# madsjulia/GeostatInversion.jl

Measured on AMD Instinct MI355X. Metric: randSVD GB/s + top-k singular-value rel-err, n=1e6 rank=256, higher is better.
Workload: dtype f64

## Files before the change

geostatinversion.jl_amd/csrc/hip_backend.hip:

```cpp
#include <hip/hip_runtime.h>
#include <rccl/rccl.h>
#include <dlfcn.h>
#include <fcntl.h>
#include <sched.h>
#include <sys/mman.h>
#include <time.h>
#include <unistd.h>
#include <algorithm>
#include <cmath>
#include <cstdlib>
#include <cstring>
#include <condition_variable>
#include <atomic>
#include <mutex>
#include <string>
#include <chrono>
#include <map>
#include <memory>
#include <set>
#include <vector>
#include "../../include/gsi_hip.h"
#include "backend.hpp"
#include "hip_common.hpp"
#include "host_staging.hpp"
// ... 368 lines not shown
      int64_t cur[3] = {1, 1, 1};
      for (int a = 0; a < d; ++a) cur[a] = 2 * p->N[a];
      int64_t tot = cur[0] * cur[1] * cur[2];
      struct Hold { HipBackend* be; double* p; ~Hold() { if (p) be->release(p); } } bufh{this, nullptr};
      bufh.p = alloc((size_t)tot);
      double*& buf = bufh.p;
      hipk::fft_spectrum_natural(st_, buf, cur, beta, 1);
      auto rotate_apply = [&](int64_t rows_out, int64_t period, bool weighted) {
        const int64_t k = cur[0], rest = (tot / k);
        Hold Bh{this, alloc((size_t)k * rows_out)};
        double* B = Bh.p;
        if (!weighted) hipk::fft_cos_matrix(st_, B, k, rows_out, period, false);
        else hipk::fft_cos_matrix(st_, B, k, rows_out, period, true);
        Hold outh{this, alloc((size_t)rest * rows_out)};
        double* out = outh.p;
        double* ws = gemm_ws(hipk::gemm_workspace_doubles(rest, rows_out, k));
        hipk::gemm_f64(st_, true, rest, rows_out, k, 1.0, buf, k, B, k, 0.0, out, rest, ws);
        check_launch("fft re-embedding product");
        release(buf);
        buf = out;
        outh.p = nullptr;
        tot = rest * rows_out;
        int64_t nd[3] = {1, 1, 1};
        for (int a = 0; a + 1 < d; ++a) nd[a] = cur[a + 1];
        nd[d - 1] = rows_out;
        for (int a = 0; a < 3; ++a) cur[a] = nd[a];
      };
      for (int a = 0; a < d; ++a) rotate_apply(p->N[a], 2 * p->N[a], false);
      for (int a = 0; a < d; ++a) rotate_apply(p->M[a], p->M[a], true);
      hipk::fft_lines_layout(st_, buf, p->lam, p->M);
      hipk::fft_finish_plan(st_, p->lam, p->lam + Mtot, p->M);
      check_launch("fft re-embedded spectrum");
      release(buf);
      buf = nullptr;
    } catch (...) {
      release(p->W); release(p->lam);
      throw;
    }
    return p.release();
  }
  void fftcov_destroy(void* plan) override {
    FftCov* p = static_cast<FftCov*>(plan);
    if (!p) return;
    release(p->W); release(p->lam);
    delete p;
  }
  void fftcov_apply(void* plan, int64_t l, const double* X, int64_t ldx, double* Y, int64_t ldy) override {
    bind();
    FftCov* p = static_cast<FftCov*>(plan);
    hipk::fft_cov_apply(st_, p->N, p->M, p->lam, reinterpret_cast<double2*>(p->W), p->nb_max, l, X, ldx, Y, ldy);
    check_launch("fft_cov_apply");
  }

  void lu_L(double* Y, int64_t m, int64_t l, int64_t ld, int32_t* ipiv_host) override {
    lu_L_impl(Y, m, l, ld, ipiv_host, nullptr);
  }
  bool lu_L_keep(double* Y, int64_t m, int64_t l, int64_t ld, int32_t** ipiv_dev) override {
    if (ipiv_dev == nullptr) return false;
    lu_L_impl(Y, m, l, ld, nullptr, ipiv_dev);
    return true;
  }
  void lu_L_impl(double* Y, int64_t m, int64_t l, int64_t ld, int32_t* ipiv_host, int32_t** ipiv_dev_out) {
    bind();
    hipk::Lu2Work w2;
    static const bool tall_first = (getenv("GSI_LU_TALL") != nullptr && getenv("GSI_LU_TALL")[0] == '1');
    static const int64_t ov_max = getenv("GSI_LU_OV_MAX") ? atoll(getenv("GSI_LU_OV_MAX")) : ((int64_t)5 << 20);
    static const bool ov_off = (getenv("GSI_LU_OV") != nullptr && getenv("GSI_LU_OV")[0] == '0');
    const bool resident_ok = !tall_first && !lu2_lost_ && ranks_sharing_device_ <= 1;
    bool fits = resident_ok && hipk::lu2_config(m, ncus_, &w2.bs, &w2.rpt, &w2.grid) && lu2_fits(w2.bs, w2.rpt, w2.grid);
    if (!fits && resident_ok && !ov_off && m <= ov_max && ncus_ >= 1) {
      const int g = std::min(ncus_, 256);
      if (m > (int64_t)g * 4096) {
        if (lu2_ov_resident_ < 0) lu2_ov_resident_ = hipk::lu2_resident_per_cu_ov();
        if ((int64_t)lu2_ov_resident_ * ncus_ >= g) { w2.bs = 512; w2.rpt = 8; w2.grid = g; w2.ov = true; fits = true; }
      }
    }
    if (fits) {
      if (const char* e = getenv("GSI_LU_POLL_LIMIT")) w2.poll_limit = atoi(e);
      if (const char* e = getenv("GSI_LU_TEST_MUTE_EPOCH")) w2.mute_epoch = (uint32_t)atoi(e);
      if (const char* e = getenv("GSI_LU_COOPERATIVE")) w2.cooperative = (e[0] == '1');
      static const int nb_env = getenv("GSI_LU_NB") ? atoi(getenv("GSI_LU_NB")) : 0;
      w2.nb = (nb_env == 32 || nb_env == 64) ? nb_env : hipk::LU2_NB;
      const size_t rec_bytes = sizeof(unsigned long long) * 2 * ((size_t)w2.grid + hipk::LU2_RES_COPIES) * hipk::LU2_REC_GRANULES;
      const size_t u12_bytes = sizeof(double) * (size_t)w2.nb * (size_t)l;
      grow(ws_lu_, rec_bytes + u12_bytes + sizeof(int32_t) * (l + 4) + 256);
      char* base = (char*)ws_lu_.p;
      w2.recs = (unsigned long long*)base; base += rec_bytes;
      w2.u12 = (double*)base; base += u12_bytes;
      w2.ipiv = (int32_t*)base;
      w2.info = flags_ + 0;
      hipk::lu2_L(st_, Y, m, l, ld, w2);
      check_launch("lu2_L");
      if (ipiv_dev_out) *ipiv_dev_out = w2.ipiv;
      if (ipiv_host) {
        HIP_CHECK(hipMemcpyAsync(ipiv_host, w2.ipiv, sizeof(int32_t) * l, hipMemcpyDeviceToHost, st_));
        HIP_CHECK(hipStreamSynchronize(st_));
      }
      return;
    }
    if (m >= ((int64_t)1 << 31)) throw Error(GSI_ERR_ARG, "lu: panels of 2^31 rows and more are not supported");
    grow(ws_lu_, hipk::lu3_work_bytes(l));
    int32_t* ipiv_dev = nullptr;
    hipk::lu3_L(st_, Y, m, l, ld, ws_lu_.p, flags_ + 0, &ipiv_dev);
    check_launch("lu3_L");
    if (ipiv_dev_out) *ipiv_dev_out = ipiv_dev;
    if (ipiv_host) {
      HIP_CHECK(hipMemcpyAsync(ipiv_host, ipiv_dev, sizeof(int32_t) * l, hipMemcpyDeviceToHost, st_));
      HIP_CHECK(hipStreamSynchronize(st_));
    }
  }
  int lus_block() const override { return hipk::LU2_NB; }
  struct LusWs { double* pval; int64_t* pidx; int32_t* ipiv; };
  LusWs lus_ws(int64_t, int64_t l) {
    if (l > 8188) throw Error(GSI_ERR_ARG, "sharded lu: sketch width too large");
    grow(ws_lus_, 32768 + 2 * 8 * 1024 + 64);
    char* base = (char*)ws_lus_.p;
    LusWs w;
    w.ipiv = (int32_t*)base;
    w.pval = (double*)(base + 32768);
    w.pidx = (int64_t*)(base + 32768 + 8 * 1024);
    return w;
  }
  void lus_u12_leaf(const double* Yloc, int64_t ld, int64_t row0, int64_t jb, int64_t j0, int w, double* U12) override {
    bind();
    hipk::lus_u12_leaf(st_, Yloc, ld, row0, jb, j0, w, U12);
    check_launch("lus_u12_leaf");
  }
  void lus_pending(double* Yloc, int64_t mloc, int64_t ld, int64_t row0, int64_t jb, int64_t j0, int w,
                   const double* U12) override {
    bind();
    if (mloc > 0) hipk::lus_pending(st_, Yloc, ld, mloc, row0, jb, j0, w, U12);
    check_launch("lus_pending");
  }
  void lus_candidate(const double* Yloc, int64_t mloc, int64_t ld, int64_t row0, int64_t l, int64_t j, double* rec) override {
    bind();
    LusWs w = lus_ws(mloc, l);
    const bool ready = (lus_part_col_ == j && lus_part_Y_ == Yloc && lus_part_mloc_ == mloc);
    lus_part_col_ = -1;
    hipk::lus_candidate(st_, Yloc, ld, mloc, row0, l, j, rec, w.pval, w.pidx, ready);
    check_launch("lus_candidate");
  }
  void lus_apply(double* Yloc, int64_t mloc, int64_t ld, int64_t row0, int64_t m, int64_t l, int64_t j0, int s, int w,
                 const double* recs, int nranks) override {
    bind();
    LusWs ws = lus_ws(mloc, l);
    static const bool fuse = (getenv("GSI_LUS_NO_FUSE") == nullptr);
    const bool next = fuse && (s + 1 < w) && mloc > 0;
    hipk::lus_apply(st_, Yloc, ld, mloc, row0, m, l, j0, s, w, recs, nranks, ws.ipiv, flags_ + 0, next ? ws.pval : nullptr,
                    next ? ws.pidx : nullptr);
    check_launch("lus_apply");
    lus_part_col_ = next ? j0 + s + 1 : -1;
    lus_part_Y_ = Yloc;
    lus_part_mloc_ = mloc;
  }
  void lus_u12_block(const double* Yloc, int64_t ld, int64_t row0, int64_t jb, int b, int64_t c0, int64_t c1,
                     double* U12) override {
    bind();
    hipk::lus_u12_block(st_, Yloc, ld, row0, jb, b, c0, c1, U12);
    check_launch("lus_u12_block");
  }
  void lus_rankk(double* Yloc, int64_t mloc, int64_t ld, int64_t row0, int64_t jb, int b, int64_t c0, int64_t t,
                 const double* U12) override {
    bind();
    hipk::lus_rankk(st_, Yloc, ld, mloc, row0, jb, b, c0, t, U12);
    check_launch("lus_rankk");
  }
  void lus_finish(double* Yloc, int64_t mloc, int64_t ld, int64_t row0, int64_t l) override {
// ... 1262 lines not shown
```

geostatinversion.jl_amd/csrc/panel_lu_leaf.hip:

```cpp
#include "hip_common.hpp"
#include <type_traits>
#include <cstdio>
#include <cstdlib>

namespace gsi { namespace hipk {

namespace {

constexpr int LW = LU2_LEAF;
constexpr int KPMAX = LU2_NB - LW;
constexpr int LSP = KPMAX + 1;
constexpr int REC = LU2_REC_GRANULES;
constexpr int POLL_LIMIT = 4000000;

__device__ inline double readlane_d(double x, int srclane) {
  int lo = __double2loint(x), hi = __double2hiint(x);
  lo = __builtin_amdgcn_readlane(lo, srclane);
  hi = __builtin_amdgcn_readlane(hi, srclane);
  return __hiloint2double(hi, lo);
}
template <int CTRL, int ROW_MASK>
__device__ inline double dpp_fmax(double v) {
  const int lo = __builtin_amdgcn_update_dpp(0, __double2loint(v), CTRL, ROW_MASK, 0xf, false);
  const int hi = __builtin_amdgcn_update_dpp((int)0xbff00000, __double2hiint(v), CTRL, ROW_MASK, 0xf, false);
// ... 651 lines not shown
    if (hit) {
#pragma unroll
      for (int rr = 0; rr < R; ++rr)
        if (grow0 + rr * BS == r) {
#pragma unroll
          for (int k = 0; k < LW; ++k) a[rr][k] = c_old[k];
        }
    }
#pragma unroll
    for (int rr = 0; rr < R; ++rr) {
      const double x0 = a[rr][s];
      const double lij = (rpiv != 0.0) ? x0 * rpiv : x0;
      a[rr][s] = lij;
#pragma unroll
      for (int k = s + 1; k < LW; ++k) a[rr][k] -= lij * u[k];
    }
    if (isdiag && tid >= s) {
      if (tid == s) {
#pragma unroll
        for (int k = 0; k < LW; ++k) d[k] = u[k];
      } else {
        if (drow == r) {
#pragma unroll
          for (int k = 0; k < LW; ++k) d[k] = c_old[k];
        }
        const double x0 = d[s];
        const double lij = (rpiv != 0.0) ? x0 * rpiv : x0;
        d[s] = lij;
#pragma unroll
        for (int k = s + 1; k < LW; ++k) d[k] -= lij * u[k];
      }
    }
    LU_STAMP(5);
  };

  {
    using std::integral_constant;
    step(integral_constant<int, 0>{});
    step(integral_constant<int, 1>{});
    step(integral_constant<int, 2>{});
    step(integral_constant<int, 3>{});
    step(integral_constant<int, 4>{});
    step(integral_constant<int, 5>{});
    step(integral_constant<int, 6>{});
    step(integral_constant<int, 7>{});
  }
  if constexpr (OV) {
    for (int32_t i = ov0; i < m; i += ovstride) {
      const int lev = ov_level(i);
      double x[LW];
#pragma unroll
      for (int k = 0; k < LW; ++k) x[k] = (k < w) ? *elem(colbase(j0 + k), i) : 0.0;
#pragma unroll
      for (int t = 0; t < LW; ++t) {
        if (t >= lev && t < w) {
          const double rp = s_rp[t];
          const double lt = (rp != 0.0) ? x[t] * rp : x[t];
          x[t] = lt;
#pragma unroll
          for (int k = t + 1; k < LW; ++k) x[k] -= lt * s_u[t * LW + k];
        }
      }
#pragma unroll
      for (int k = 0; k < LW; ++k) if (k < w) *elem(colbase(j0 + k), i) = x[k];
    }
  }
  if (s_abort && tid == 0) atomicExch(info, -1);
  if (has_col && pend) { swcol[pj] = pa1; swcol[pr] = pa0; }
#pragma unroll
  for (int k = 0; k < LW; ++k) {
    if (k < w) {
      char* cb = colbase(j0 + k);
#pragma unroll
      for (int rr = 0; rr < R; ++rr) {
        const int32_t i = row0 + rr * BS;
        if (i < m) *elem(cb, i) = a[rr][k];
      }
      if (isdiag && drow < m) *elem(cb, drow) = d[k];
    }
  }
}

template <int K>
__global__ __launch_bounds__(256) void lu_u12_kernel(const double* __restrict__ Y, int64_t ld, int64_t jb, int64_t jbrow,
                                                     int64_t c0, int64_t c1, double* __restrict__ out) {
  __shared__ double L11[K * K];
#pragma unroll 8
  for (int e = threadIdx.x; e < K * K; e += 256) {
    const int r = e % K, c = e / K;
    L11[r * K + c] = Y[(jbrow + r) + (jb + c) * ld];
  }
  __syncthreads();
  if (threadIdx.x >= 64) return;
  const int64_t c = c0 + (int64_t)blockIdx.x * 64 + threadIdx.x;
  if (c >= c1) return;
  double x[K];
  const double* col = Y + jbrow + c * ld;
#pragma unroll
  for (int r = 0; r < K; ++r) x[r] = col[r];
#pragma unroll
  for (int r = 1; r < K; ++r) {
    double v = x[r];
#pragma unroll
    for (int p = 0; p < r; ++p) v -= L11[r * K + p] * x[p];
    x[r] = v;
  }
  double* o = out + (c - c0) * K;
#pragma unroll
  for (int r = 0; r < K; ++r) o[r] = x[r];
}

template <int K, int DEPTH, int RK_CHUNK>
__global__ __launch_bounds__(256) __attribute__((amdgpu_waves_per_eu(RK_CHUNK == 64 ? 3 : 2, RK_CHUNK == 64 ? 3 : 4))) void lu_rankk_kernel(double* __restrict__ Y, int64_t ld, int64_t m, int64_t r_begin,
                                                       int64_t jb, int64_t c0, int64_t t,
                                                       const double* __restrict__ U12) {
  typedef double double4_t __attribute__((ext_vector_type(4)));
  constexpr int KP = K + 2;
  extern __shared__ double us[];
  const int tid = threadIdx.x, lane = tid & 63, wave = tid >> 6;
  const int jl = lane & 15, kk = lane >> 4;
  const int64_t rb = r_begin + ((int64_t)blockIdx.x * 4 + wave) * 32;
  double fa[2][K / 4];
#pragma unroll
  for (int h = 0; h < 2; ++h) {
    const int64_t rrow = rb + 16 * h + jl;
#pragma unroll
    for (int s = 0; s < K / 4; ++s) fa[h][s] = (rrow < m) ? Y[rrow + (jb + 4 * s + kk) * ld] : 0.0;
  }
  for (int64_t cc0 = 0; cc0 < t; cc0 += RK_CHUNK) {
    const int tc = (int)((t - cc0 < RK_CHUNK) ? (t - cc0) : RK_CHUNK);
    __syncthreads();
    for (int e = tid; e < RK_CHUNK * K; e += 256) {
      const int k = e % K, c = e / K;
      us[c * KP + k] = (c < tc) ? U12[k + (cc0 + c) * K] : 0.0;
    }
    __syncthreads();
    if (rb >= m) continue;
    const int ntile = (tc + 15) / 16;
    double cin[2][4];
    auto load_tile = [&](int tt, double (&dst)[2][4]) {
#pragma unroll
      for (int h = 0; h < 2; ++h) {
        const int64_t rrow = rb + 16 * h + jl;
#pragma unroll
        for (int reg = 0; reg < 4; ++reg) {
          const int cl = 16 * tt + kk + 4 * reg;
          dst[h][reg] = (rrow < m && cl < tc) ? Y[rrow + (c0 + cc0 + cl) * ld] : 0.0;
        }
      }
    };
    load_tile(0, cin);
    double cin2[2][4];
    if (DEPTH == 2 && ntile > 1) load_tile(1, cin2);
    for (int tt = 0; tt < ntile; ++tt) {
      double4_t acc[2];
#pragma unroll
      for (int h = 0; h < 2; ++h) acc[h] = (double4_t){cin[h][0], cin[h][1], cin[h][2], cin[h][3]};
      if (DEPTH == 2) {
#pragma unroll
        for (int h = 0; h < 2; ++h)
#pragma unroll
          for (int reg = 0; reg < 4; ++reg) cin[h][reg] = cin2[h][reg];
        if (tt + 2 < ntile) load_tile(tt + 2, cin2);
      } else if (tt + 1 < ntile) load_tile(tt + 1, cin);
#pragma unroll
      for (int s = 0; s < K / 4; ++s) {
        const double fb = -us[(16 * tt + jl) * KP + 4 * s + kk];
#pragma unroll
        for (int h = 0; h < 2; ++h) acc[h] = __builtin_amdgcn_mfma_f64_16x16x4f64(fb, fa[h][s], acc[h], 0, 0, 0);
      }
#pragma unroll
      for (int h = 0; h < 2; ++h) {
        const int64_t rrow = rb + 16 * h + jl;
#pragma unroll
        for (int reg = 0; reg < 4; ++reg) {
          const int cl = 16 * tt + kk + 4 * reg;
          if (rrow < m && cl < tc) Y[rrow + (c0 + cc0 + cl) * ld] = acc[h][reg];
        }
      }
    }
  }
}

template <int K, int DEPTH, int CHUNK>
static void launch_rankk_v(hipStream_t st, unsigned grid, double* Y, int64_t ld, int64_t m, int64_t r_begin, int64_t jb,
                           int64_t c0, int64_t t, const double* U12) {
  constexpr size_t shmem = (size_t)CHUNK * (K + 2) * sizeof(double);
  static std::atomic<uint64_t> attr_mask{0};
  if (first_use_on_this_device(attr_mask))
    (void)hipFuncSetAttribute((const void*)lu_rankk_kernel<K, DEPTH, CHUNK>, hipFuncAttributeMaxDynamicSharedMemorySize, (int)shmem);
  hipLaunchKernelGGL((lu_rankk_kernel<K, DEPTH, CHUNK>), dim3(grid), dim3(256), shmem, st, Y, ld, m, r_begin, jb, c0, t, U12);
}
template <int K>
static void launch_rankk(hipStream_t st, unsigned grid, double* Y, int64_t ld, int64_t m, int64_t r_begin, int64_t jb,
                         int64_t c0, int64_t t, const double* U12) {
  static const int depth = getenv("GSI_LU_RK_DEPTH") ? atoi(getenv("GSI_LU_RK_DEPTH")) : 1;
  static const int chunk = getenv("GSI_LU_RK_CHUNK") ? atoi(getenv("GSI_LU_RK_CHUNK")) : 64;
  if (chunk == 64 && depth == 2) launch_rankk_v<K, 2, 64>(st, grid, Y, ld, m, r_begin, jb, c0, t, U12);
  else if (chunk == 64) launch_rankk_v<K, 1, 64>(st, grid, Y, ld, m, r_begin, jb, c0, t, U12);
  else if (depth == 2) launch_rankk_v<K, 2, 128>(st, grid, Y, ld, m, r_begin, jb, c0, t, U12);
  else launch_rankk_v<K, 1, 128>(st, grid, Y, ld, m, r_begin, jb, c0, t, U12);
}

__global__ void lu2_extract_L_kernel(double* __restrict__ Y, int64_t ld, int64_t l) {
  const int64_t total = l * l;
  for (int64_t e = (int64_t)blockIdx.x * blockDim.x + threadIdx.x; e < total; e += (int64_t)gridDim.x * blockDim.x) {
    const int64_t r = e % l, c = e / l;
    if (r == c) Y[r + c * ld] = 1.0;
    else if (r < c) Y[r + c * ld] = 0.0;
  }
}

bool lu2_config(int64_t m, int ncus, int* bs, int* rpt, int* grid) {
  if (ncus < 1) return false;
  if (ncus > 256) ncus = 256;
  static const int cfg[4][2] = {{256, 1}, {256, 4}, {512, 4}, {512, 8}};
  for (int c = 0; c < 4; ++c) {
    const int64_t per = (int64_t)cfg[c][0] * cfg[c][1];
    if (m <= (int64_t)ncus * per) { *bs = cfg[c][0]; *rpt = cfg[c][1]; *grid = (int)((m + per - 1) / per); return true; }
  }
  return false;
}

template <int BS, int R>
static void launch_leaf(hipStream_t st, int grid, double* Y, int64_t ld, int64_t m, int64_t l, int64_t jb, int64_t j0,
                        int w, const Lu2Work& wk, uint32_t epoch_base) {
  static const int onehop = getenv("GSI_LU_ONEHOP") ? atoi(getenv("GSI_LU_ONEHOP")) : 1;
  const int poll_limit = wk.poll_limit > 0 ? wk.poll_limit : POLL_LIMIT;
  LuMrArgs none{};
  if constexpr (BS == 512 && R == 8) {
    if (wk.ov) {
      hipLaunchKernelGGL((lu_leaf_kernel<512, 8, false, true>), dim3(grid), dim3(512), 0, st, Y, ld, (int32_t)m, (int32_t)l,
                         (int32_t)jb, (int32_t)j0, w, wk.recs, epoch_base, wk.ipiv, wk.info, 1, poll_limit, wk.mute_epoch, none);
      return;
    }
  }
  if (!wk.cooperative) {
    hipLaunchKernelGGL((lu_leaf_kernel<BS, R, false>), dim3(grid), dim3(BS), 0, st, Y, ld, (int32_t)m, (int32_t)l, (int32_t)jb,
                       (int32_t)j0, w, wk.recs, epoch_base, wk.ipiv, wk.info, onehop, poll_limit, wk.mute_epoch, none);
    return;
  }
  int32_t m32 = (int32_t)m, l32 = (int32_t)l, jb32 = (int32_t)jb, j032 = (int32_t)j0;
  int oh = onehop, pl = poll_limit;
  uint32_t eb = epoch_base, mute = wk.mute_epoch;
  unsigned long long* recs = wk.recs;
  int32_t* ipiv = wk.ipiv;
  int32_t* info = wk.info;
  void* args[] = {&Y, &ld, &m32, &l32, &jb32, &j032, &w, &recs, &eb, &ipiv, &info, &oh, &pl, &mute, &none};
  (void)hipLaunchCooperativeKernel((const void*)lu_leaf_kernel<BS, R, false>, dim3(grid), dim3(BS), args, 0, st);
}

template <int BS, int R>
static int leaf_resident_per_cu() {
  int nblk = 0;
  if (hipOccupancyMaxActiveBlocksPerMultiprocessor(&nblk, (const void*)lu_leaf_kernel<BS, R, false>, BS, 0) != hipSuccess) {
    (void)hipGetLastError();
    return 0;
  }
  return nblk;
}
int lu2_resident_per_cu_ov() {
  int nblk = 0;
  if (hipOccupancyMaxActiveBlocksPerMultiprocessor(&nblk, (const void*)lu_leaf_kernel<512, 8, false, true>, 512, 0) != hipSuccess) {
    (void)hipGetLastError();
    return 0;
  }
  return nblk;
}
int lu2_resident_per_cu(int bs, int rpt) {
  if (bs == 256 && rpt == 1) return leaf_resident_per_cu<256, 1>();
  if (bs == 256) return leaf_resident_per_cu<256, 4>();
  if (rpt == 4) return leaf_resident_per_cu<512, 4>();
  return leaf_resident_per_cu<512, 8>();
}

bool lu2_mr_config(int64_t pad, int nranks, int ncus, int* bs, int* rpt, int* grid, int* hier, int* ov, int force) {
  *ov = 0;
  if (nranks < 1 || nranks > LU2_MAX_RANKS) return false;
  if (force == 2) {
    if (nranks < 2 || pad <= 2 * 4096 || ncus < 2) return false;
    *bs = 512; *rpt = 8; *grid = 2; *hier = 1; *ov = 1;
    return true;
  }
  static const int ov_cap = getenv("GSI_LU_MR_OV_GRID") ? atoi(getenv("GSI_LU_MR_OV_GRID")) : 0;
// ... 171 lines not shown
        v[t] = Y[(srow[t] - row0) + c * ld];
        const unsigned long long bits = (unsigned long long)__double_as_longlong(v[t]);
        const size_t off = box_off + ((size_t)t * lq + (size_t)c) * 2;
        for (int q = 0; q < mr.nranks; ++q) {
          if (q == mr.rank) continue;
          __hip_atomic_store(mr.peer[q] + off, ((unsigned long long)tag << 32) | (uint32_t)bits, __ATOMIC_RELAXED, __HIP_MEMORY_SCOPE_SYSTEM);
          __hip_atomic_store(mr.peer[q] + off + 1, ((unsigned long long)tag << 32) | (uint32_t)(bits >> 32), __ATOMIC_RELAXED,
                             __HIP_MEMORY_SCOPE_SYSTEM);
        }
      }
    }
    {
      unsigned long long lo[2 * LW], hi[2 * LW];
      int tries = timed_out ? poll_limit : 0;
      for (;;) {
        bool ok = true;
#pragma unroll
        for (int t = 0; t < 2 * LW; ++t) {
          if (scan[t] && !smine[t]) {
            const size_t off = box_off + ((size_t)t * lq + (size_t)c) * 2;
            lo[t] = poll_granule<true>(own + off);
            hi[t] = poll_granule<true>(own + off + 1);
          }
        }
#pragma unroll
        for (int t = 0; t < 2 * LW; ++t)
          if (scan[t] && !smine[t]) ok = ok && ((uint32_t)(lo[t] >> 32) == tag && (uint32_t)(hi[t] >> 32) == tag);
        if (ok) break;
        if (++tries > poll_limit) { timed_out = true; lu_timeout_note(info, 6, (int)c, tag, mr.rank * 1024 + (int)blockIdx.x); break; }
        __builtin_amdgcn_s_sleep(1);
      }
#pragma unroll
      for (int t = 0; t < 2 * LW; ++t)
        if (scan[t] && !smine[t])
          v[t] = __longlong_as_double((long long)(((unsigned long long)(uint32_t)hi[t] << 32) | (uint32_t)lo[t]));
    }
    for (int s2 = 0; s2 < w; ++s2) {
      const int b = lus_swap_slot_lw(piv, w, j0, piv[s2]);
      if (b >= 0 && b != s2) {
        double va = 0.0, vb = 0.0;
#pragma unroll
        for (int t = 0; t < 2 * LW; ++t) { if (t == s2) va = v[t]; if (t == b) vb = v[t]; }
#pragma unroll
        for (int t = 0; t < 2 * LW; ++t) { if (t == s2) v[t] = vb; if (t == b) v[t] = va; }
      }
    }
#pragma unroll
    for (int t = 0; t < 2 * LW; ++t)
      if (smine[t]) Y[(srow[t] - row0) + c * ld] = v[t];
  }
  if (timed_out) atomicExch(info, -1);
}
void lus_swap_peer(hipStream_t st, const Lu2MrWork& w, double* Y, int64_t ld, int64_t mloc, int64_t row0, int64_t m, int64_t l,
                   int64_t j0, int wd, uint32_t epoch_base) {
  LuMrArgs a{};
  a.rank = w.rank; a.nranks = w.nranks; a.gbase = (int32_t)row0; a.mtot = (int32_t)m; a.us = nullptr;
  for (int q = 0; q < w.nranks; ++q) a.peer[q] = w.peer[q];
  const int64_t pad = (m + w.nranks - 1) / w.nranks;
  const size_t G = w.hier ? (size_t)w.grid + (size_t)w.nranks : (size_t)w.nranks * (size_t)w.grid;
  const size_t box = (size_t)2 * G * REC + (size_t)2 * (2 * KPMAX * LW) + (size_t)((epoch_base >> 3) & 1u) * ((size_t)2 * LW * 2 * LU2_MR_MAXL);
  const int poll_limit = w.poll_limit > 0 ? w.poll_limit : POLL_LIMIT;
  const int g = (int)std::min<int64_t>((l + 255) / 256, 64);
  hipLaunchKernelGGL(lus_swap_peer_kernel, dim3(g), dim3(256), 0, st, Y, ld, mloc, row0, l, (int32_t)j0, wd, w.ipiv, a, w.peer[w.rank], box,
                     epoch_base + 1u, pad, poll_limit, w.info);
}

void lus_swap_pack(hipStream_t st, const double* Y, int64_t ld, int64_t mloc, int64_t row0, int64_t l, int64_t j0, int w,
                   const int32_t* ipiv, double* table) {
  const int g = (int)std::min<int64_t>((2 * LW * l + 255) / 256, 256);
  hipLaunchKernelGGL(lus_swap_pack_kernel, dim3(g), dim3(256), 0, st, Y, ld, mloc, row0, l, (int32_t)j0, w, ipiv, table);
}
void lus_swap_apply(hipStream_t st, double* Y, int64_t ld, int64_t mloc, int64_t row0, int64_t l, int64_t j0, int w,
                    const int32_t* ipiv, const double* table) {
  const int g = (int)std::min<int64_t>((l + 255) / 256, 64);
  hipLaunchKernelGGL(lus_swap_apply_kernel, dim3(g), dim3(256), 0, st, Y, ld, mloc, row0, l, (int32_t)j0, w, ipiv, table);
}

void lu2_L(hipStream_t st, double* Y, int64_t m, int64_t l, int64_t ld, const Lu2Work& w) {
  (void)hipMemsetAsync(w.recs, 0, sizeof(unsigned long long) * 2 * ((size_t)w.grid + LU2_RES_COPIES) * REC, st);
  uint32_t epoch = 0;
  const int nb = w.nb;
  for (int64_t jb = 0; jb < l; jb += nb) {
    const int b = (int)((l - jb < nb) ? (l - jb) : nb);
    for (int64_t j0 = jb; j0 < jb + b; j0 += LW) {
      const int wd = (int)((jb + b - j0 < LW) ? (jb + b - j0) : LW);
      if (w.bs == 256 && w.rpt == 1) launch_leaf<256, 1>(st, w.grid, Y, ld, m, l, jb, j0, wd, w, epoch);
      else if (w.bs == 256) launch_leaf<256, 4>(st, w.grid, Y, ld, m, l, jb, j0, wd, w, epoch);
      else if (w.rpt == 4) launch_leaf<512, 4>(st, w.grid, Y, ld, m, l, jb, j0, wd, w, epoch);
      else launch_leaf<512, 8>(st, w.grid, Y, ld, m, l, jb, j0, wd, w, epoch);
      epoch += (uint32_t)LW;
    }
    const int64_t c0 = jb + b, t = l - c0;
    if (t > 0) {
      const int64_t mr = m - c0;
      const unsigned gu = (unsigned)((t + 63) / 64);
      const unsigned gr = (unsigned)((mr + 127) / 128);
      if (b == 64) {
        hipLaunchKernelGGL(lu_u12_kernel<64>, dim3(gu), dim3(256), 0, st, Y, ld, jb, jb, c0, l, w.u12);
        if (mr > 0) launch_rankk<64>(st, gr, Y, ld, m, c0, jb, c0, t, w.u12);
      } else {
        hipLaunchKernelGGL(lu_u12_kernel<32>, dim3(gu), dim3(256), 0, st, Y, ld, jb, jb, c0, l, w.u12);
        if (mr > 0) launch_rankk<32>(st, gr, Y, ld, m, c0, jb, c0, t, w.u12);
      }
    }
  }
  int eb = (int)((l * l + 255) / 256);
  if (eb > 1024) eb = 1024;
  hipLaunchKernelGGL(lu2_extract_L_kernel, dim3(eb), dim3(256), 0, st, Y, ld, l);
#ifdef GSI_LU_TRACE
  if (const char* path = getenv("GSI_LU_TRACE")) {
    unsigned long long h[4 * 8 * 8];
    (void)hipStreamSynchronize(st);
    (void)hipMemcpyFromSymbol(h, HIP_SYMBOL(g_lu_trace), sizeof(h));
    if (FILE* f = fopen(path, "w")) {
      for (int tw = 0; tw < 4; ++tw)
        for (int s = 0; s < 8; ++s) {
          fprintf(f, "wg%d step%d", tw, s);
          for (int ph = 0; ph < 6; ++ph) fprintf(f, " %llu", h[(tw * 8 + s) * 8 + ph]);
          fprintf(f, "\n");
        }
      fclose(f);
    }
  }
#endif
}

namespace {
constexpr int T_BS = 256;
constexpr int T_R = 4;
constexpr int T_MAXWG = 4096;
struct Lu3State {
  double u[LW][LW];
  double rp[LW];
};

struct Lu3Step {
  double* Y;
  int64_t ld, m;
  int32_t l, j0;
  int s, w;
  double* pval;
  int64_t* pidx;
  Lu3State* stt;
  int32_t* ipiv;
  int32_t* info;
};
__device__ inline void lu3_step_tail(double best, int32_t besti, const Lu3Step& p) {
  __shared__ double s_v[T_BS / 64];
  __shared__ int32_t s_i[T_BS / 64];
  const int tid = threadIdx.x, lane = tid & 63, wave = tid >> 6;
  wave_argmax(best, besti);
  if (lane == 0) { s_v[wave] = best; s_i[wave] = besti; }
  __syncthreads();
  if (tid == 0) {
    double bv = -1.0;
    int32_t bi = -1;
    for (int q = 0; q < T_BS / 64; ++q)
      if (s_i[q] >= 0 && (s_v[q] > bv || (s_v[q] == bv && s_i[q] < bi))) { bv = s_v[q]; bi = s_i[q]; }
    p.pval[blockIdx.x] = bv;
    p.pidx[blockIdx.x] = bi;
  }
}
__global__ __launch_bounds__(T_BS) void lu3_pivot_kernel(Lu3Step p, int nwg) {
  __shared__ double s_v[T_BS / 64];
  __shared__ int32_t s_i[T_BS / 64];
  __shared__ double s_x[LW];
  const int tid = threadIdx.x, lane = tid & 63, wave = tid >> 6;
  double best = -1.0;
  int32_t besti = -1;
  for (int e = tid; e < nwg; e += T_BS) {
    const double v = p.pval[e];
    const int32_t i = (int32_t)p.pidx[e];
    if (i >= 0 && (v > best || (v == best && i < besti))) { best = v; besti = i; }
  }
  wave_argmax(best, besti);
  if (lane == 0) { s_v[wave] = best; s_i[wave] = besti; }
  __syncthreads();
  double bestv = -1.0;
  int32_t r = -1;
  for (int q = 0; q < T_BS / 64; ++q)
    if (s_i[q] >= 0 && (s_v[q] > bestv || (s_v[q] == bestv && s_i[q] < r))) { bestv = s_v[q]; r = s_i[q]; }
  double* const Y = p.Y;
  const int64_t ld = p.ld;
  const int32_t j0 = p.j0, j = p.j0 + p.s;
  const int s = p.s, w = p.w;
  const bool valid = (r >= j && (int64_t)r < p.m);
  if (!valid) r = j;
// ... 187 lines not shown
  const int64_t stride = (int64_t)gridDim.x * (T_BS * T_R);
  for (int64_t base = (int64_t)j0 + S1 + (int64_t)blockIdx.x * (T_BS * T_R) + threadIdx.x; base < m; base += stride) {
    double x[T_R][S1 + 1];
#pragma unroll
    for (int k = 0; k <= S1; ++k) {
      const double* cb = Y + (int64_t)(j0 + k) * ld;
#pragma unroll
      for (int rr = 0; rr < T_R; ++rr) {
        const int64_t i = base + rr * T_BS;
        x[rr][k] = (i < m) ? cb[i] : 0.0;
      }
    }
#pragma unroll
    for (int rr = 0; rr < T_R; ++rr) {
#pragma unroll
      for (int t = 0; t < S1; ++t) {
        const double lt = (rp[t] != 0.0) ? x[rr][t] * rp[t] : x[rr][t];
#pragma unroll
        for (int k = t + 1; k <= S1; ++k) x[rr][k] -= lt * u[t][k];
      }
      const int64_t i = base + rr * T_BS;
      const double av = fabs(x[rr][S1]);
      if (i < m && av > best) { best = av; besti = (int32_t)i; }
    }
  }
  lu3_step_tail(best, besti, p);
}

__global__ __launch_bounds__(T_BS) void lu3_close_kernel(double* __restrict__ Y, int64_t ld, int64_t m, int32_t j0, int w,
                                                         const Lu3State* stt) {
  double u[LW][LW], rp[LW];
#pragma unroll
  for (int t = 0; t < LW; ++t) {
    rp[t] = stt->rp[t];
#pragma unroll
    for (int k = t + 1; k < LW; ++k) u[t][k] = stt->u[t][k];
  }
  const int64_t stride = (int64_t)gridDim.x * (T_BS * T_R);
  for (int64_t base = (int64_t)j0 + w + (int64_t)blockIdx.x * (T_BS * T_R) + threadIdx.x; base < m; base += stride) {
    double x[T_R][LW];
#pragma unroll
    for (int k = 0; k < LW; ++k) {
      const double* cb = Y + (int64_t)(j0 + (k < w ? k : 0)) * ld;
#pragma unroll
      for (int rr = 0; rr < T_R; ++rr) {
        const int64_t i = base + rr * T_BS;
        x[rr][k] = (i < m && k < w) ? cb[i] : 0.0;
      }
    }
#pragma unroll
    for (int rr = 0; rr < T_R; ++rr) {
#pragma unroll
      for (int t = 0; t < LW; ++t) {
        if (t < w) {
          const double lt = (rp[t] != 0.0) ? x[rr][t] * rp[t] : x[rr][t];
          x[rr][t] = lt;
#pragma unroll
          for (int k = t + 1; k < LW; ++k) x[rr][k] -= lt * u[t][k];
        }
      }
    }
#pragma unroll
    for (int k = 0; k < LW; ++k) {
      if (k < w) {
        double* cb = Y + (int64_t)(j0 + k) * ld;
#pragma unroll
        for (int rr = 0; rr < T_R; ++rr) {
          const int64_t i = base + rr * T_BS;
          if (i < m) cb[i] = x[rr][k];
        }
      }
    }
  }
}

static int lu3_grid(int64_t rows) {
  const int64_t per = (int64_t)T_BS * T_R;
  const int64_t g = (rows + per - 1) / per;
  return (int)std::max<int64_t>(1, std::min<int64_t>(g, T_MAXWG));
}
}

size_t lu3_work_bytes(int64_t l) {
  return sizeof(double) * T_MAXWG + sizeof(int64_t) * T_MAXWG + sizeof(Lu3State) + sizeof(double) * (size_t)LU2_NB * (size_t)l +
         sizeof(int32_t) * (size_t)(l + 4) + 512;
}

void lu3_L(hipStream_t st, double* Y, int64_t m, int64_t l, int64_t ld, void* work, int32_t* info, int32_t** ipiv_out) {
  char* base = (char*)work;
  double* pval = (double*)base; base += sizeof(double) * T_MAXWG;
  int64_t* pidx = (int64_t*)base; base += sizeof(int64_t) * T_MAXWG;
  Lu3State* stt = (Lu3State*)base; base += sizeof(Lu3State);
  double* u12 = (double*)base; base += sizeof(double) * (size_t)LU2_NB * (size_t)l;
  int32_t* ipiv = (int32_t*)base;
  *ipiv_out = ipiv;
  const int nb = LU2_NB;
  static const bool fuse = !(getenv("GSI_LU_TALL_NOFUSE") != nullptr);
  for (int64_t jb = 0; jb < l; jb += nb) {
    const int b = (int)((l - jb < nb) ? (l - jb) : nb);
    for (int64_t j0 = jb; j0 < jb + b; j0 += LW) {
      const int wd = (int)((jb + b - j0 < LW) ? (jb + b - j0) : LW);
      Lu3Step p{Y, ld, m, (int32_t)l, (int32_t)j0, 0, wd, pval, pidx, stt, ipiv, info};
      const int g = lu3_grid(m - j0);
      if (j0 == jb) hipLaunchKernelGGL((lu3_open_kernel<false, false>), dim3(g), dim3(T_BS), 0, st, (int32_t)jb, p);
      else if (fuse) hipLaunchKernelGGL((lu3_open_kernel<true, true>), dim3(g), dim3(T_BS), 0, st, (int32_t)jb, p);
      else hipLaunchKernelGGL((lu3_open_kernel<true, false>), dim3(g), dim3(T_BS), 0, st, (int32_t)jb, p);
      hipLaunchKernelGGL(lu3_pivot_kernel, dim3(1), dim3(T_BS), 0, st, p, g);
      for (int s1 = 1; s1 < wd; ++s1) {
        p.s = s1;
        const int gc = lu3_grid(m - j0 - s1);
        switch (s1) {
          case 1: hipLaunchKernelGGL(lu3_cand_kernel<1>, dim3(gc), dim3(T_BS), 0, st, p); break;
          case 2: hipLaunchKernelGGL(lu3_cand_kernel<2>, dim3(gc), dim3(T_BS), 0, st, p); break;
          case 3: hipLaunchKernelGGL(lu3_cand_kernel<3>, dim3(gc), dim3(T_BS), 0, st, p); break;
          case 4: hipLaunchKernelGGL(lu3_cand_kernel<4>, dim3(gc), dim3(T_BS), 0, st, p); break;
          case 5: hipLaunchKernelGGL(lu3_cand_kernel<5>, dim3(gc), dim3(T_BS), 0, st, p); break;
          case 6: hipLaunchKernelGGL(lu3_cand_kernel<6>, dim3(gc), dim3(T_BS), 0, st, p); break;
          default: hipLaunchKernelGGL(lu3_cand_kernel<7>, dim3(gc), dim3(T_BS), 0, st, p); break;
        }
        hipLaunchKernelGGL(lu3_pivot_kernel, dim3(1), dim3(T_BS), 0, st, p, gc);
      }
      const bool next_opens = fuse && (j0 + wd < jb + b);
      if (m > j0 + wd && !next_opens)
        hipLaunchKernelGGL(lu3_close_kernel, dim3(lu3_grid(m - j0 - wd)), dim3(T_BS), 0, st, Y, ld, m, (int32_t)j0, wd, stt);
    }
    const int64_t c0 = jb + b, t = l - c0;
    if (t > 0) {
      const int64_t mr = m - c0;
      const unsigned gu = (unsigned)((t + 63) / 64);
      const unsigned gr = (unsigned)((mr + 127) / 128);
      hipLaunchKernelGGL(lu_u12_kernel<64>, dim3(gu), dim3(256), 0, st, Y, ld, jb, jb, c0, l, u12);
      if (mr > 0) launch_rankk<64>(st, gr, Y, ld, m, c0, jb, c0, t, u12);
    }
  }
  int eb = (int)((l * l + 255) / 256);
  if (eb > 1024) eb = 1024;
  hipLaunchKernelGGL(lu2_extract_L_kernel, dim3(eb), dim3(256), 0, st, Y, ld, l);
}

namespace {
constexpr int LUS_HDR = 4;

__global__ __launch_bounds__(256) void lus_cand_partial_kernel(const double* __restrict__ Y, int64_t ld, int64_t mloc,
                                                               int64_t row0, int64_t j, double* __restrict__ pval,
                                                               int64_t* __restrict__ pidx) {
  __shared__ double s_v[4];
  __shared__ int32_t s_i[4];
  double best = -1.0;
  int32_t besti = -1;
  for (int64_t li = (int64_t)blockIdx.x * 256 + threadIdx.x; li < mloc; li += (int64_t)gridDim.x * 256) {
    const int64_t gi = row0 + li;
    if (gi >= j) {
      const double av = fabs(Y[li + j * ld]);
      if (av > best) { best = av; besti = (int32_t)gi; }
    }
  }
  wave_argmax(best, besti);
  if ((threadIdx.x & 63) == 0) { s_v[threadIdx.x >> 6] = best; s_i[threadIdx.x >> 6] = besti; }
  __syncthreads();
  if (threadIdx.x < 64) {
    double v = (threadIdx.x < 4) ? s_v[threadIdx.x] : -1.0;
    int32_t i = (threadIdx.x < 4) ? s_i[threadIdx.x] : -1;
    wave_argmax8(v, i);
    if (threadIdx.x == 0) { pval[blockIdx.x] = v; pidx[blockIdx.x] = i; }
  }
}
__global__ __launch_bounds__(256) void lus_cand_final_kernel(const double* __restrict__ Y, int64_t ld, int64_t mloc,
                                                             int64_t row0, int64_t l, int64_t j, int nparts,
                                                             const double* __restrict__ pval, const int64_t* __restrict__ pidx,
                                                             double* __restrict__ rec) {
  __shared__ double s_v[4];
  __shared__ int32_t s_i[4];
  __shared__ int32_t s_win;
  double best = -1.0;
  int32_t besti = -1;
  for (int p = threadIdx.x; p < nparts; p += 256) {
    const double v = pval[p];
    const int32_t i = (int32_t)pidx[p];
    if (v > best || (v == best && (uint32_t)i < (uint32_t)besti)) { best = v; besti = i; }
  }
  wave_argmax(best, besti);
  if ((threadIdx.x & 63) == 0) { s_v[threadIdx.x >> 6] = best; s_i[threadIdx.x >> 6] = besti; }
  __syncthreads();
  if (threadIdx.x < 64) {
    double v = (threadIdx.x < 4) ? s_v[threadIdx.x] : -1.0;
    int32_t i = (threadIdx.x < 4) ? s_i[threadIdx.x] : -1;
    wave_argmax8(v, i);
    if (threadIdx.x == 0) {
      s_win = i;
      rec[0] = v;
      rec[1] = (double)i;
      rec[2] = (j >= row0 && j < row0 + mloc) ? 1.0 : 0.0;
      rec[3] = 0.0;
    }
  }
  __syncthreads();
  const int64_t wi = s_win;
  const bool has_j = (j >= row0 && j < row0 + mloc);
  for (int64_t c = threadIdx.x; c < l; c += 256) {
    rec[LUS_HDR + c] = (wi >= 0) ? Y[(wi - row0) + c * ld] : 0.0;
    rec[LUS_HDR + l + c] = has_j ? Y[(j - row0) + c * ld] : 0.0;
  }
}

__global__ __launch_bounds__(256) void lus_apply_kernel(double* __restrict__ Y, int64_t ld, int64_t mloc, int64_t row0,
                                                        int64_t m, int64_t l, int64_t j0, int s, int w,
                                                        const double* __restrict__ recs, int nranks,
                                                        int32_t* __restrict__ ipiv, int32_t* __restrict__ info,
                                                        double* __restrict__ pval, int64_t* __restrict__ pidx) {
  __shared__ double s_v4[4];
  __shared__ int32_t s_i4[4];
  __shared__ double s_u[LW], s_old[LW];
  __shared__ int32_t s_r;
  __shared__ int s_gw, s_go;
  __shared__ double s_bestv;
  const int64_t j = j0 + s;
// ... 192 lines not shown
```

Measured before the change: 1601.

## Switch blocked panel LU from right-looking to left-looking trailing updates

```diff
diff --git a/geostatinversion.jl_amd/csrc/hip_backend.hip b/geostatinversion.jl_amd/csrc/hip_backend.hip
--- a/geostatinversion.jl_amd/csrc/hip_backend.hip
+++ b/geostatinversion.jl_amd/csrc/hip_backend.hip
@@ -474,7 +474,7 @@
       static const int nb_env = getenv("GSI_LU_NB") ? atoi(getenv("GSI_LU_NB")) : 0;
       w2.nb = (nb_env == 32 || nb_env == 64) ? nb_env : hipk::LU2_NB;
       const size_t rec_bytes = sizeof(unsigned long long) * 2 * ((size_t)w2.grid + hipk::LU2_RES_COPIES) * hipk::LU2_REC_GRANULES;
-      const size_t u12_bytes = sizeof(double) * (size_t)w2.nb * (size_t)l;
+      const size_t u12_bytes = sizeof(double) * (size_t)l * (size_t)l;
       grow(ws_lu_, rec_bytes + u12_bytes + sizeof(int32_t) * (l + 4) + 256);
       char* base = (char*)ws_lu_.p;
       w2.recs = (unsigned long long*)base; base += rec_bytes;
diff --git a/geostatinversion.jl_amd/csrc/panel_lu_leaf.hip b/geostatinversion.jl_amd/csrc/panel_lu_leaf.hip
--- a/geostatinversion.jl_amd/csrc/panel_lu_leaf.hip
+++ b/geostatinversion.jl_amd/csrc/panel_lu_leaf.hip
@@ -757,14 +757,29 @@
 }
 
 template <int K>
-__global__ __launch_bounds__(256) void lu_u12_kernel(const double* __restrict__ Y, int64_t ld, int64_t jb, int64_t jbrow,
-                                                     int64_t c0, int64_t c1, double* __restrict__ out) {
-  __shared__ double L11[K * K];
+__device__ inline void u12_stage_L11(double* L11, const double* __restrict__ Y, int64_t ld, int64_t jb, int64_t jbrow) {
 #pragma unroll 8
   for (int e = threadIdx.x; e < K * K; e += 256) {
     const int r = e % K, c = e / K;
     L11[r * K + c] = Y[(jbrow + r) + (jb + c) * ld];
   }
+}
+template <int K>
+__device__ inline void u12_solve(const double* L11, double (&x)[K]) {
+#pragma unroll
+  for (int r = 1; r < K; ++r) {
+    double v = x[r];
+#pragma unroll
+    for (int p = 0; p < r; ++p) v -= L11[r * K + p] * x[p];
+    x[r] = v;
+  }
+}
+
+template <int K>
+__global__ __launch_bounds__(256) void lu_u12_kernel(const double* __restrict__ Y, int64_t ld, int64_t jb, int64_t jbrow,
+                                                     int64_t c0, int64_t c1, double* __restrict__ out) {
+  __shared__ double L11[K * K];
+  u12_stage_L11<K>(L11, Y, ld, jb, jbrow);
   __syncthreads();
   if (threadIdx.x >= 64) return;
   const int64_t c = c0 + (int64_t)blockIdx.x * 64 + threadIdx.x;
@@ -773,13 +788,7 @@
   const double* col = Y + jbrow + c * ld;
 #pragma unroll
   for (int r = 0; r < K; ++r) x[r] = col[r];
-#pragma unroll
-  for (int r = 1; r < K; ++r) {
-    double v = x[r];
-#pragma unroll
-    for (int p = 0; p < r; ++p) v -= L11[r * K + p] * x[p];
-    x[r] = v;
-  }
+  u12_solve<K>(L11, x);
   double* o = out + (c - c0) * K;
 #pragma unroll
   for (int r = 0; r < K; ++r) o[r] = x[r];
@@ -875,6 +884,190 @@
   else if (chunk == 64) launch_rankk_v<K, 1, 64>(st, grid, Y, ld, m, r_begin, jb, c0, t, U12);
   else if (depth == 2) launch_rankk_v<K, 2, 128>(st, grid, Y, ld, m, r_begin, jb, c0, t, U12);
   else launch_rankk_v<K, 1, 128>(st, grid, Y, ld, m, r_begin, jb, c0, t, U12);
+}
+
+constexpr int LL_WAVES = 12;
+constexpr int LL_BS = 64 * LL_WAVES;
+constexpr size_t LL_LDS = (size_t)4 * 64 * 66 * sizeof(double);
+template <int NB>
+constexpr int ll_group() { return (int)(LL_LDS / ((size_t)NB * (NB + 2) * sizeof(double))); }
+
+__device__ __forceinline__ char* ll_advance(char* p, int64_t step) {
+  p += step;
+  asm volatile("" : "+s"(p));
+  return p;
+}
+
+template <int NB, bool WIDE>
+__global__ __launch_bounds__(LL_BS) void lu_leftlook_kernel(double* __restrict__ Y, int64_t ld, int64_t m, int64_t jb, int tc,
+                                                            int ip0, int ip1, const double* __restrict__ U12, int64_t ldu) {
+  typedef double double4_t __attribute__((ext_vector_type(4)));
+  typedef typename std::conditional<WIDE, uint64_t, uint32_t>::type off_t;
+  constexpr int KP = NB + 2, NT = NB / 16, NS = NB / 4;
+  extern __shared__ double us[];
+  const int tid = threadIdx.x, lane = tid & 63;
+  const int wave = __builtin_amdgcn_readfirstlane(tid >> 6);
+  const int jl = lane & 15, kk = lane >> 4;
+  const int nbk = ip1 - ip0;
+  for (int e = tid; e < nbk * NB * NB; e += LL_BS) {
+    const int k = e % NB, c = (e / NB) % NB, q = e / (NB * NB);
+    us[(q * NB + c) * KP + k] = (c < tc) ? -U12[(int64_t)(ip0 + q) * ldu + (jb + c) * NB + k] : 0.0;
+  }
+  __syncthreads();
+  const int lb = jl * KP + kk;
+  const int64_t nch = (m - jb + 15) / 16;
+  const int64_t cs = ld * (int64_t)sizeof(double);
+  for (int64_t ch = (int64_t)blockIdx.x * LL_WAVES + wave; ch < nch; ch += (int64_t)gridDim.x * LL_WAVES) {
+    const int64_t rb = jb + ch * 16;
+    const int64_t r = (rb + jl < m) ? rb + jl : m - 1;
+    const off_t vo = (off_t)((r - rb) * (int64_t)sizeof(double) + kk * cs);
+    auto at = [&](char* colp) -> double* { return reinterpret_cast<double*>(colp + vo); };
+    char* const cbase = reinterpret_cast<char*>(Y + rb + jb * ld);
+    double4_t acc[NT];
+    {
+      char* p = cbase;
+#pragma unroll
+      for (int tt = 0; tt < NT; ++tt)
+#pragma unroll
+        for (int reg = 0; reg < 4; ++reg) {
+          acc[tt][reg] = (16 * tt + 4 * reg + kk < tc) ? *at(p) : 0.0;
+          p = ll_advance(p, 4 * cs);
+        }
+    }
+    double fa[NS], fn[NS];
+    char* pf = reinterpret_cast<char*>(Y + rb + (int64_t)ip0 * NB * ld);
+    auto load_frag = [&](double (&f)[NS]) {
+#pragma unroll
+      for (int s = 0; s < NS; ++s) {
+        f[s] = *at(pf);
+        pf = ll_advance(pf, 4 * cs);
+      }
+    };
+    auto run = [&](const double (&f)[NS], int q) {
+      const double* ub = us + (q - ip0) * NB * KP + lb;
+#pragma unroll
+      for (int s = 0; s < NS; ++s)
+#pragma unroll
+        for (int tt = 0; tt < NT; ++tt)
+          acc[tt] = __builtin_amdgcn_mfma_f64_16x16x4f64(ub[16 * tt * KP + 4 * s], f[s], acc[tt], 0, 0, 0);
+    };
+    load_frag(fa);
+    int q = ip0;
+    for (; q + 1 < ip1; ++q) {
+      load_frag(fn);
+      run(fa, q);
+#pragma unroll
+      for (int s = 0; s < NS; ++s) fa[s] = fn[s];
+    }
+    run(fa, q);
+    const bool live = rb + jl < m;
+    char* p = cbase;
+#pragma unroll
+    for (int tt = 0; tt < NT; ++tt)
+#pragma unroll
+      for (int reg = 0; reg < 4; ++reg) {
+        if (live && 16 * tt + 4 * reg + kk < tc) *at(p) = acc[tt][reg];
+        p = ll_advance(p, 4 * cs);
+      }
+  }
+}
+
+template <int K>
+__global__ __launch_bounds__(256) void lu_urows_kernel(const double* __restrict__ Y, int64_t ld, int64_t jb, int nprev,
+                                                       int64_t c0, int64_t c1, const double* __restrict__ U12, int64_t ldu,
+                                                       double* __restrict__ out) {
+  typedef double double4_t __attribute__((ext_vector_type(4)));
+  constexpr int TP = K + 1;
+  __shared__ double L11[K * K];
+  __shared__ double T[64 * TP];
+  u12_stage_L11<K>(L11, Y, ld, jb, jb);
+  const int tid = threadIdx.x, lane = tid & 63, wave = tid >> 6;
+  const int jl = lane & 15, kk = lane >> 4;
+  const int64_t cb = c0 + (int64_t)blockIdx.x * 64;
+  if (wave < K / 16) {
+    const int64_t row = jb + 16 * wave + jl;
+    double4_t acc[4];
+#pragma unroll
+    for (int tt = 0; tt < 4; ++tt)
+#pragma unroll
+      for (int reg = 0; reg < 4; ++reg) {
+        const int64_t c = cb + 16 * tt + kk + 4 * reg;
+        acc[tt][reg] = (c < c1) ? Y[row + c * ld] : 0.0;
+      }
+    for (int q = 0; q < nprev; ++q) {
+      const double* ub = U12 + (int64_t)q * ldu;
+#pragma unroll
+      for (int s = 0; s < K / 4; ++s) {
+        const double fa = Y[row + ((int64_t)q * K + 4 * s + kk) * ld];
+#pragma unroll
+        for (int tt = 0; tt < 4; ++tt) {
+          const int64_t c = cb + 16 * tt + jl;
+          const double fb = (c < c1) ? -ub[c * K + 4 * s + kk] : 0.0;
+          acc[tt] = __builtin_amdgcn_mfma_f64_16x16x4f64(fb, fa, acc[tt], 0, 0, 0);
+        }
+      }
+    }
+#pragma unroll
+    for (int tt = 0; tt < 4; ++tt)
+#pragma unroll
+      for (int reg = 0; reg < 4; ++reg) T[(16 * tt + kk + 4 * reg) * TP + 16 * wave + jl] = acc[tt][reg];
+  }
+  __syncthreads();
+  if (tid >= 64) return;
+  const int64_t c = cb + tid;
+  if (c >= c1) return;
+  double x[K];
+#pragma unroll
+  for (int r = 0; r < K; ++r) x[r] = T[tid * TP + r];
+  u12_solve<K>(L11, x);
+  double* o = out + (c - c0) * K;
+#pragma unroll
+  for (int r = 0; r < K; ++r) o[r] = x[r];
+}
+
+template <int NB, bool WIDE>
+static void launch_leftlook_v(hipStream_t st, unsigned grid, double* Y, int64_t ld, int64_t m, int64_t jb, int tc,
+                              const double* U12, int64_t ldu) {
+  static std::atomic<uint64_t> attr_mask{0};
+  if (first_use_on_this_device(attr_mask))
+    (void)hipFuncSetAttribute((const void*)lu_leftlook_kernel<NB, WIDE>, hipFuncAttributeMaxDynamicSharedMemorySize, (int)LL_LDS);
+  const int nprev = (int)(jb / NB);
+  for (int ip0 = 0; ip0 < nprev; ip0 += ll_group<NB>()) {
+    const int ip1 = std::min(nprev, ip0 + ll_group<NB>());
+    const size_t shmem = (size_t)(ip1 - ip0) * NB * (NB + 2) * sizeof(double);
+    hipLaunchKernelGGL((lu_leftlook_kernel<NB, WIDE>), dim3(grid), dim3(LL_BS), shmem, st, Y, ld, m, jb, tc, ip0, ip1, U12, ldu);
+  }
+}
+static void lu_ll_update(hipStream_t st, double* Y, int64_t ld, int64_t m, int64_t l, int64_t jb, int b, int nb,
+                         const double* u12) {
+  if (jb == 0 || m <= jb) return;
+  int dev = 0, ncu = 0;
+  (void)hipGetDevice(&dev);
+  if (hipDeviceGetAttribute(&ncu, hipDeviceAttributeMultiprocessorCount, dev) != hipSuccess || ncu < 1) ncu = 256;
+  const int64_t chunks = (m - jb + 15) / 16;
+  const unsigned grid = (unsigned)std::min<int64_t>((chunks + LL_WAVES - 1) / LL_WAVES, ncu);
+  const bool wide = (3 * ld + 32) * (int64_t)sizeof(double) >= ((int64_t)1 << 32);
+  const int64_t ldu = (int64_t)nb * l;
+  if (nb == 64) {
+    if (wide) launch_leftlook_v<64, true>(st, grid, Y, ld, m, jb, b, u12, ldu);
+    else launch_leftlook_v<64, false>(st, grid, Y, ld, m, jb, b, u12, ldu);
+  } else {
+    if (wide) launch_leftlook_v<32, true>(st, grid, Y, ld, m, jb, b, u12, ldu);
+    else launch_leftlook_v<32, false>(st, grid, Y, ld, m, jb, b, u12, ldu);
+  }
+}
+static void lu_ll_urows(hipStream_t st, const double* Y, int64_t ld, int64_t l, int64_t jb, int nb, double* u12) {
+  const int64_t c0 = jb + nb, ldu = (int64_t)nb * l;
+  if (c0 >= l) return;
+  const unsigned gu = (unsigned)((l - c0 + 63) / 64);
+  double* out = u12 + (jb / nb) * ldu + c0 * nb;
+  if (nb == 64) {
+    if (jb == 0) hipLaunchKernelGGL(lu_u12_kernel<64>, dim3(gu), dim3(256), 0, st, Y, ld, jb, jb, c0, l, out);
+    else hipLaunchKernelGGL(lu_urows_kernel<64>, dim3(gu), dim3(256), 0, st, Y, ld, jb, (int)(jb / nb), c0, l, u12, ldu, out);
+  } else {
+    if (jb == 0) hipLaunchKernelGGL(lu_u12_kernel<32>, dim3(gu), dim3(256), 0, st, Y, ld, jb, jb, c0, l, out);
+    else hipLaunchKernelGGL(lu_urows_kernel<32>, dim3(gu), dim3(256), 0, st, Y, ld, jb, (int)(jb / nb), c0, l, u12, ldu, out);
+  }
 }
 
 __global__ void lu2_extract_L_kernel(double* __restrict__ Y, int64_t ld, int64_t l) {
@@ -1212,6 +1405,7 @@
   const int nb = w.nb;
   for (int64_t jb = 0; jb < l; jb += nb) {
     const int b = (int)((l - jb < nb) ? (l - jb) : nb);
+    lu_ll_update(st, Y, ld, m, l, jb, b, nb, w.u12);
     for (int64_t j0 = jb; j0 < jb + b; j0 += LW) {
       const int wd = (int)((jb + b - j0 < LW) ? (jb + b - j0) : LW);
       if (w.bs == 256 && w.rpt == 1) launch_leaf<256, 1>(st, w.grid, Y, ld, m, l, jb, j0, wd, w, epoch);
@@ -1220,19 +1414,7 @@
       else launch_leaf<512, 8>(st, w.grid, Y, ld, m, l, jb, j0, wd, w, epoch);
       epoch += (uint32_t)LW;
     }
-    const int64_t c0 = jb + b, t = l - c0;
-    if (t > 0) {
-      const int64_t mr = m - c0;
-      const unsigned gu = (unsigned)((t + 63) / 64);
-      const unsigned gr = (unsigned)((mr + 127) / 128);
-      if (b == 64) {
-        hipLaunchKernelGGL(lu_u12_kernel<64>, dim3(gu), dim3(256), 0, st, Y, ld, jb, jb, c0, l, w.u12);
-        if (mr > 0) launch_rankk<64>(st, gr, Y, ld, m, c0, jb, c0, t, w.u12);
-      } else {
-        hipLaunchKernelGGL(lu_u12_kernel<32>, dim3(gu), dim3(256), 0, st, Y, ld, jb, jb, c0, l, w.u12);
-        if (mr > 0) launch_rankk<32>(st, gr, Y, ld, m, c0, jb, c0, t, w.u12);
-      }
-    }
+    lu_ll_urows(st, Y, ld, l, jb, nb, w.u12);
   }
   int eb = (int)((l * l + 255) / 256);
   if (eb > 1024) eb = 1024;
@@ -1586,7 +1768,7 @@
 }
 
 size_t lu3_work_bytes(int64_t l) {
-  return sizeof(double) * T_MAXWG + sizeof(int64_t) * T_MAXWG + sizeof(Lu3State) + sizeof(double) * (size_t)LU2_NB * (size_t)l +
+  return sizeof(double) * T_MAXWG + sizeof(int64_t) * T_MAXWG + sizeof(Lu3State) + sizeof(double) * (size_t)l * (size_t)l +
          sizeof(int32_t) * (size_t)(l + 4) + 512;
 }
 
@@ -1595,13 +1777,14 @@
   double* pval = (double*)base; base += sizeof(double) * T_MAXWG;
   int64_t* pidx = (int64_t*)base; base += sizeof(int64_t) * T_MAXWG;
   Lu3State* stt = (Lu3State*)base; base += sizeof(Lu3State);
-  double* u12 = (double*)base; base += sizeof(double) * (size_t)LU2_NB * (size_t)l;
+  double* u12 = (double*)base; base += sizeof(double) * (size_t)l * (size_t)l;
   int32_t* ipiv = (int32_t*)base;
   *ipiv_out = ipiv;
   const int nb = LU2_NB;
   static const bool fuse = !(getenv("GSI_LU_TALL_NOFUSE") != nullptr);
   for (int64_t jb = 0; jb < l; jb += nb) {
     const int b = (int)((l - jb < nb) ? (l - jb) : nb);
+    lu_ll_update(st, Y, ld, m, l, jb, b, nb, u12);
     for (int64_t j0 = jb; j0 < jb + b; j0 += LW) {
       const int wd = (int)((jb + b - j0 < LW) ? (jb + b - j0) : LW);
       Lu3Step p{Y, ld, m, (int32_t)l, (int32_t)j0, 0, wd, pval, pidx, stt, ipiv, info};
@@ -1628,14 +1811,7 @@
       if (m > j0 + wd && !next_opens)
         hipLaunchKernelGGL(lu3_close_kernel, dim3(lu3_grid(m - j0 - wd)), dim3(T_BS), 0, st, Y, ld, m, (int32_t)j0, wd, stt);
     }
-    const int64_t c0 = jb + b, t = l - c0;
-    if (t > 0) {
-      const int64_t mr = m - c0;
-      const unsigned gu = (unsigned)((t + 63) / 64);
-      const unsigned gr = (unsigned)((mr + 127) / 128);
-      hipLaunchKernelGGL(lu_u12_kernel<64>, dim3(gu), dim3(256), 0, st, Y, ld, jb, jb, c0, l, u12);
-      if (mr > 0) launch_rankk<64>(st, gr, Y, ld, m, c0, jb, c0, t, u12);
-    }
+    lu_ll_urows(st, Y, ld, l, jb, nb, u12);
   }
   int eb = (int)((l * l + 255) / 256);
   if (eb > 1024) eb = 1024;
```

After: 1635 (median of 6 runs). +2.1%, better.
